# PaddlePaddle/Parakeet

Hardware: AMD Instinct MI355X
Metric: audio samples/sec, FastSpeech2+PWGAN 22.05kHz (higher is better)
Workload: dtype f32 (3-term split-fp16 MFMA, fp32-equivalent; exact-fp32 in roofline.exact_f32); 1 GPU; FastSpeech2+PWG end-to-end (BASELINE config 4 per-GPU share): 32 utterances/GPU x 128 phonemes -> 640 frames -> 163840 samples each, LJSpeech architecture, random-init weights; utterances_per_gpu=32, global_batch=32, minibatch=32, parallelism=dp1 (utterance sharding, no data-path collective)

## Files before the change

parakeet_amd/csrc/ffn_planes.hip:

```cpp
#include "pk_ffn_planes.h"

#include <algorithm>
#include <cmath>
#include <cstdlib>
#include <cstring>

#include "pk_mfma.h"
#include "pk_split.h"

namespace {
constexpr int ROW_B = 16, LO_OFF = 512;

struct Args {
    FfnpConv c;
    int active;
    int nrg;
    int nct;
    long in_blk, out_blk;
};

__device__ __forceinline__ unsigned pow2_neg_h2(int d) {
    const float f = __uint_as_float((unsigned)(127 - min(d, 60)) << 23);
    return __builtin_bit_cast(unsigned, __builtin_amdgcn_cvt_pkrtz(f, f));
}
__device__ __forceinline__ f16x8 h8_of(unsigned u) {
    const u32x4 v = {u, u, u, u};
    return __builtin_bit_cast(f16x8, v);
}

template <int NQ, int KQ, int EPI, int W, int TAPS = FFNP_TAPS, int ABL = 0, bool BF32 = false, int CPT = 6, int ACT = 0>
__global__ __launch_bounds__(64 * W, 2) void k_ffn_planes(Args a) {
    constexpr int THREADS = 64 * W;
    constexpr int HT = TAPS / 2;
    constexpr int SLAB_CH = CPT * THREADS;
    constexpr int KCH = 2 * NQ * 64;
    constexpr int SLAB = SLAB_CH / KCH;
    constexpr int nks = TAPS * KQ;
    constexpr int G = nks / SLAB;
    constexpr int RING = NQ >= 6 ? 6 : 9;
    constexpr bool TIGHT = NQ == 8;
    static_assert(SLAB_CH % KCH == 0 && nks % SLAB == 0 && nks > RING && G >= 3, "shape");
    static_assert(!BF32 || (TAPS == 1 && !TIGHT), "fp32 operand: one tap, the untight loop");
    __shared__ __attribute__((aligned(16))) f16x8 wbuf[3][SLAB_CH];
    __shared__ __attribute__((aligned(16))) float lb[32 * NQ];
    __shared__ float lbs[NQ];
    const int tid = threadIdx.x, lane = tid & 63, wave = tid >> 6;
    const int j = lane & 31, hh = lane >> 5;
    const int xcd = (int)blockIdx.x & 7, k = (int)blockIdx.x >> 3;
    const int rg = (k / a.nct) * 8 + xcd, ct = k % a.nct;
    if (rg >= a.nrg) return;
    for (int i = tid; i < 32 * NQ; i += THREADS) {
        const int h2 = i / (16 * NQ), q = (i / 16) % NQ, r = i % 16;
        lb[i] = a.c.bias ? a.c.bias[ct * (32 * NQ) + 32 * q + mfma_row(r, h2)] : 0.f;
    }
    if (tid < NQ) lbs[tid] = a.c.wscale[ct * NQ + tid];
    const f16x8* wt = reinterpret_cast<const f16x8*>(a.c.w) + (long)ct * ((long)G * SLAB_CH) + tid;
    const int blk = rg * a.active + wave;
    const bool tile_ok = wave < a.active && blk < a.c.nblk;
    f16x8 wreg[CPT];

    if (tile_ok) {
        const int p = blk * FFNP_BLK + j;
        const int rv = a.c.row_utt[p];
        unsigned am[TAPS];
#pragma unroll
        for (int t = 0; t < TAPS; ++t) am[t] = a.c.in_amax[p + t - HT];
        const char* inb = reinterpret_cast<const char*>(a.c.in) + ((long)blk - 1) * a.in_blk;
        unsigned off[TAPS];
#pragma unroll
        for (int t = 0; t < TAPS; ++t) {
            const int q = j + t - HT;
            off[t] = (unsigned)((q + 32) >> 5) * (unsigned)a.in_blk + (unsigned)((q & 31) * ROW_B + hh * 1024);
        }
        f16x8 rhi[RING], rlo[RING];
        auto load_b = [&](int ks) {
            const int kq = ks / TAPS, tap = ks % TAPS, slot = ks % RING;
            if (BF32) {
                const float* src = reinterpret_cast<const float*>(a.c.in) + (long)p * a.c.ldin + 16 * kq + 4 * hh;
                rhi[slot] = ld_h8(reinterpret_cast<const char*>(src));
                rlo[slot] = ld_h8(reinterpret_cast<const char*>(src + 8));
                return;
            }
            const char* src = inb + (off[tap] + (unsigned)(kq * 2048));
            rhi[slot] = ld_h8(src);
            rlo[slot] = ld_h8(src + LO_OFF);
        };
        {
            f16x8 wreg1[CPT];
#pragma unroll
            for (int c = 0; c < CPT; ++c) wreg[c] = wt[c * THREADS];
#pragma unroll
            for (int c = 0; c < CPT; ++c) wreg1[c] = wt[SLAB_CH + c * THREADS];
#pragma unroll
            for (int kk = 0; kk < RING; ++kk) load_b(kk);
            __builtin_amdgcn_sched_barrier(0);
#pragma unroll
            for (int c = 0; c < CPT; ++c) wbuf[0][c * THREADS + tid] = wreg[c];
#pragma unroll
            for (int c = 0; c < CPT; ++c) wbuf[1][c * THREADS + tid] = wreg1[c];
        }
        int ex = amax_exp(am[0]);
#pragma unroll
        for (int t = 1; t < TAPS; ++t) ex = max(ex, amax_exp(am[t]));
        const int kx = PK_BLK_TOP + 127 - ex;
        const float sx = pow2f(kx);
        unsigned fu[TAPS];
#pragma unroll
        for (int t = 0; t < TAPS; ++t) fu[t] = pow2_neg_h2(ex - amax_exp(am[t]));
        f32x16 acc[NQ];
#pragma unroll
        for (int q = 0; q < NQ; ++q)
#pragma unroll
            for (int r = 0; r < 16; ++r) acc[q][r] = 0.f;
        __syncthreads();
#pragma unroll
        for (int g = 0; g < G; ++g) {
            const int NW = g + 2 >= G ? 0 : CPT, HW = TIGHT ? NW / 2 : NW;
#pragma unroll
            for (int c = 0; c < CPT; ++c)
                if (c < HW && !(ABL & (8 | 256))) wreg[c] = wt[(long)(g + 2) * SLAB_CH + c * THREADS];
            __builtin_amdgcn_sched_barrier(0);
            unsigned wo = (g % 3) * SLAB_CH + lane;
            asm volatile("" : "+v"(wo));
            const f16x8* wl = &wbuf[0][0] + wo;
#pragma unroll
            for (int kk = 0; kk < SLAB; ++kk) {
                const int ks = SLAB * g + kk, slot = ks % RING;
                const f16x8 f = h8_of(fu[ks % TAPS]);
                f16x8 bh, bl;
                if (TIGHT) {
                    rhi[slot] *= f;
                    rlo[slot] *= f;
                } else {
                    if (BF32) {
                        const f32x4 v0 = __builtin_bit_cast(f32x4, rhi[slot]), v1 = __builtin_bit_cast(f32x4, rlo[slot]);
                        float v[8];
#pragma unroll
                        for (int e = 0; e < 4; ++e) {
                            v[e] = rv >= 0 ? v0[e] * sx : 0.f;
                            v[4 + e] = rv >= 0 ? v1[e] * sx : 0.f;
                        }
                        split8(v, bh, bl);
                    } else {
                        bh = TAPS == 1 ? rhi[slot] : rhi[slot] * f;
                        bl = TAPS == 1 ? rlo[slot] : rlo[slot] * f;
                    }
                    __builtin_amdgcn_sched_barrier(0);
                    if (!(ABL & 1) && ks + RING < nks) load_b(ks + RING);
                }
                __builtin_amdgcn_sched_barrier(0);
// ... 6 lines not shown
                    acc[q] = mfma16(ah, TIGHT ? rlo[slot] : bl, acc[q]);
                }
                constexpr int AHEAD = NQ == 8 ? 1 : 2;
                __builtin_amdgcn_sched_group_barrier(0x100, 2 * AHEAD, 0);
#pragma unroll
                for (int q = 0; q < NQ; ++q) {
                    if (q + AHEAD < NQ) __builtin_amdgcn_sched_group_barrier(0x100, 2, 0);
                    __builtin_amdgcn_sched_group_barrier(0x008, 3, 0);
                }
                if (TIGHT) {
                    __builtin_amdgcn_sched_barrier(0);
                    if (!(ABL & 1) && ks + RING < nks) load_b(ks + RING);
                    if (kk == 0 && NW > 0 && !(ABL & 8)) {
#pragma unroll
                        for (int c = 0; c < CPT; ++c)
                            if (c < HW) wbuf[(g + 2) % 3][c * THREADS + tid] = wreg[c];
#pragma unroll
                        for (int c = 0; c < CPT; ++c)
                            if (c < NW - HW) wreg[c] = wt[(long)(g + 2) * SLAB_CH + (HW + c) * THREADS];
                    }
                    __builtin_amdgcn_sched_barrier(0);
                }
            }
#pragma unroll
            for (int c = 0; c < CPT; ++c)
                if (c < (TIGHT ? NW - HW : NW) && !(ABL & 8)) {
                    if (ABL & 128) {
                        unsigned keep = __builtin_bit_cast(u32x4, wreg[c])[0];
                        asm volatile("" : "+v"(keep));
                    } else {
                        wbuf[(g + 2) % 3][((TIGHT ? HW : 0) + c) * THREADS + tid] = wreg[c];
                    }
                }
            __syncthreads();
        }
        const float pinv = pow2f(-kx);
        const f32x4* lb4 = reinterpret_cast<const f32x4*>(lb) + hh * (NQ * 4);
        if (EPI == 0) {
            float m3 = __uint_as_float(am[0]);
#pragma unroll
            for (int t = 1; t < TAPS; ++t) m3 = fmaxf(m3, __uint_as_float(am[t]));
            const float hb = fmaf(m3, a.c.c1, a.c.c0);
            const float so = pow2f(blk_scale_exp(__float_as_uint(hb)));
            char* dst = reinterpret_cast<char*>(a.c.out) + (long)blk * a.out_blk + (long)(ct * NQ * 2) * 2048 + j * ROW_B + hh * 1024;
            const bool row_ok = rv >= 0;
#pragma unroll
            for (int q = 0; q < NQ; ++q)
#pragma unroll
                for (int m = 0; m < 2; ++m) {
                    float v[8];
#pragma unroll
                    for (int i = 0; i < 2; ++i) {
                        const f32x4 b4 = lb4[q * 4 + 2 * m + i];
#pragma unroll
                        for (int e = 0; e < 4; ++e) {
                            const float pre = fmaf(acc[q][8 * m + 4 * i + e], pinv * lbs[q], b4[e]);
                            const float t = ACT == 1 ? tanhf(pre) : fmaxf(pre, 0.f);
                            v[4 * i + e] = row_ok ? t : 0.f;
                        }
                    }
                    f16x8 oh, ol;
                    store_pair8(v, so, oh, ol);
                    if ((ABL & 4) && oh[0] != (_Float16)12345.f) continue;
                    st_h8(dst + (2 * q + m) * 2048, oh);
                    st_h8(dst + (2 * q + m) * 2048 + LO_OFF, ol);
                }
            if (ct == 0 && hh == 0) a.c.out_amax[p] = row_ok ? __float_as_uint(hb) : 0u;
// ... 1 lines not shown
            float* yr = a.c.x + (long)p * a.c.ldx + ct * (32 * NQ) + 4 * hh;
#pragma unroll
            for (int q = 0; q < NQ; ++q)
#pragma unroll
                for (int i = 0; i < 4; ++i) {
                    const f32x4 b4 = lb4[q * 4 + i];
                    f32x4 o;
#pragma unroll
                    for (int e = 0; e < 4; ++e) {
                        const float pre = fmaf(acc[q][4 * i + e], pinv * lbs[q], b4[e]);
                        o[e] = ACT == 0 ? pre : (rv >= 0 ? (ACT == 1 ? tanhf(pre) : fmaxf(pre, 0.f)) : 0.f);
                    }
                    *reinterpret_cast<f32x4*>(yr + 32 * q + 8 * i) = o;
                }
        } else {
            float* xr = a.c.x + (long)p * a.c.ldx + ct * (32 * NQ) + 4 * hh;
            f32x4 old[NQ][4];
#pragma unroll
            for (int q = 0; q < NQ; ++q)
#pragma unroll
                for (int i = 0; i < 4; ++i) old[q][i] = (ABL & 4) ? f32x4{0.f, 0.f, 0.f, 0.f} : *reinterpret_cast<const f32x4*>(xr + 32 * q + 8 * i);
#pragma unroll
            for (int q = 0; q < NQ; ++q)
#pragma unroll
                for (int i = 0; i < 4; ++i) {
                    const f32x4 b4 = lb4[q * 4 + i];
                    f32x4 o;
#pragma unroll
                    for (int e = 0; e < 4; ++e) o[e] = old[q][i][e] + fmaf(acc[q][4 * i + e], pinv * lbs[q], b4[e]);
                    if ((ABL & 4) && o[0] != 12345.f) continue;
                    *reinterpret_cast<f32x4*>(xr + 32 * q + 8 * i) = o;
                }
        }
    } else {
#pragma unroll
        for (int c = 0; c < CPT; ++c) wbuf[0][c * THREADS + tid] = wt[c * THREADS];
#pragma unroll
        for (int c = 0; c < CPT; ++c) wbuf[1][c * THREADS + tid] = wt[SLAB_CH + c * THREADS];
        __syncthreads();
#pragma unroll 1
        for (int g = 0; g < G; ++g) {
            if (g + 2 < G) {
#pragma unroll
                for (int c = 0; c < CPT; ++c) wreg[c] = wt[(long)(g + 2) * SLAB_CH + c * THREADS];
#pragma unroll
                for (int c = 0; c < CPT; ++c) wbuf[(g + 2) % 3][c * THREADS + tid] = wreg[c];
            }
            __syncthreads();
        }
    }
}

__global__ __launch_bounds__(256) void k_ffn_ln_planes(const float* __restrict__ x, const float* __restrict__ g,
                                                      const float* __restrict__ b, const int* __restrict__ row_utt, int C,
                                                      float eps, char* __restrict__ out, unsigned* __restrict__ out_amax) {
    const int blk = blockIdx.x, wave = threadIdx.x >> 6, lane = threadIdx.x & 63;
    const int noct = C >> 3;
    const bool on = lane < noct;
    const int kq = lane >> 1, hh = lane & 1;
    const int c0 = 16 * kq + 4 * hh;
    const bool ident = g == nullptr;
    f32x4 ga = {0.f, 0.f, 0.f, 0.f}, gb = ga, ba = ga, bb = ga;
    if (on && !ident) {
        ga = *reinterpret_cast<const f32x4*>(g + c0);
        gb = *reinterpret_cast<const f32x4*>(g + c0 + 8);
        ba = *reinterpret_cast<const f32x4*>(b + c0);
// ... 136 lines not shown
            uint16_t* base = dst + ((size_t)ct * nks + ks) * (2 * nq * 64 * 8);
            for (int q = 0; q < nq; ++q)
                for (int lane = 0; lane < 64; ++lane)
                    for (int e = 0; e < 8; ++e) {
                        const int i = lane & 31, hh = lane >> 5;
                        const int co = ct * 32 * nq + 32 * q + i;
                        const int ci = 16 * kq + 8 * (e >> 2) + 4 * hh + (e & 3);
                        const float w = std::ldexp(kn[((size_t)tap * Cin + ci) * N + co], kw[co / 32]);
                        const uint16_t h = f32_to_f16_rne(w);
                        base[((size_t)(0 * nq + q) * 64 + lane) * 8 + e] = h;
                        base[((size_t)(1 * nq + q) * 64 + lane) * 8 + e] = f32_to_f16_rne(w - f16_to_f32(h));
                    }
        }
    return off;
}

template <bool PROF, class Go>
static int ffnp_ablation(Go& go, bool shape_ok) {
    if constexpr (PROF) {
        static const int abl = pk_prof_env("PK_FFNP_ABLATE") ? atoi(pk_prof_env("PK_FFNP_ABLATE")) : 0;
        if (abl && shape_ok) {
            switch (abl) {
                case 1: return go(k_ffn_planes<4, 96, 1, 4, FFNP_TAPS, 1>);
                case 4: return go(k_ffn_planes<4, 96, 1, 4, FFNP_TAPS, 4>);
                case 8: return go(k_ffn_planes<4, 96, 1, 4, FFNP_TAPS, 8>);
                case 13: return go(k_ffn_planes<4, 96, 1, 4, FFNP_TAPS, 13>);
                case 128: return go(k_ffn_planes<4, 96, 1, 4, FFNP_TAPS, 128>);
                case 256: return go(k_ffn_planes<4, 96, 1, 4, FFNP_TAPS, 256>);
                default: PK_FAIL(PK_EINVAL, "PK_FFNP_ABLATE: 1, 4, 8, 13, 128 or 256 (with PK_FFNP_VARIANT=84)");
            }
        }
    }
    return 1;
}

int ffnp_conv_launch(pk_ctx* ctx, const char* prof_name, const FfnpConv& c) {
    const bool first = c.out != nullptr;
    if (!(first ? (c.Cin == 384 && c.N % (32 * FFNP_NQ1) == 0) : (c.Cin == 1536 && c.N % (32 * FFNP_NQ2) == 0)) || c.nblk <= 0 || !c.w || !c.wscale)
        PK_FAIL(PK_EINVAL, "ffnp_conv_launch: shape (Cin %d, N %d) not built", c.Cin, c.N);
    const int variant = c.variant;
    const bool one = c.w1 && variant == 0 && (long)c.nblk * (c.N / 32) <= c.one_max;
    const bool small = !one && first && c.w4 && (variant / 10 == 4 || (variant / 10 != 8 && c.nblk < FFNP_NQ1_MIN_BLOCKS));
    const int nq = one ? 1 : (first && !small ? FFNP_NQ1 : FFNP_NQ2);
    const int W = one ? 8 : (first ? (small ? 4 : 8) : (variant % 10 == 4 ? 4 : 8));
    Args a;
    a.c = c;
    if (small) a.c.w = c.w4;
    if (one) a.c.w = c.w1;
    a.nct = c.N / (32 * nq);
    a.in_blk = (long)c.Cin * 128;
    a.out_blk = (long)c.N * 128;
    int active = W;
    if (W == 8)
        while (active > 2 && (long)pk_div_up(c.nblk, active) * a.nct < ctx->n_cu) active >>= 1;
    a.active = active;
    a.nrg = pk_div_up(c.nblk, active);
    const int grid = pk_div_up(a.nrg, 8) * 8 * a.nct;
    auto go = [&](auto kern) -> int {
        PK_LAUNCH(ctx, prof_name, kern, dim3(grid), dim3(64 * W), 0, a);
        return PK_OK;
    };
    if (int st = ffnp_ablation<PK_PROFILE_BUILD != 0>(go, !first && W == 4); st != 1) return st;
    if (one) return first ? go(k_ffn_planes<1, 24, 0, 8>) : go(k_ffn_planes<1, 96, 1, 8>);
    if (first) return small ? go(k_ffn_planes<FFNP_NQ2, 24, 0, 4>) : go(k_ffn_planes<FFNP_NQ1, 24, 0, 8>);
    return W == 8 ? go(k_ffn_planes<FFNP_NQ2, 96, 1, 8>) : go(k_ffn_planes<FFNP_NQ2, 96, 1, 4>);
}

int ffnp_linear_launch(pk_ctx* ctx, const char* prof_name, const FfnpConv& c) {
    const int nq = c.ldin ? FFNP_NQ2 : FFNP_NQL;
    if (c.Cin != 384 || c.N % (32 * nq) != 0 || c.nblk <= 0 || !c.w || !c.wscale || !c.x)
        PK_FAIL(PK_EINVAL, "ffnp_linear_launch: shape (Cin %d, N %d) not built", c.Cin, c.N);
    Args a;
    a.c = c;
    a.nct = c.N / (32 * nq);
    a.in_blk = (long)c.Cin * 128;
    a.out_blk = 0;
    int active = 8;
    while (active > 2 && (long)pk_div_up(c.nblk, active) * a.nct < ctx->n_cu) active >>= 1;
    a.active = active;
    a.nrg = pk_div_up(c.nblk, active);
    const int grid = pk_div_up(a.nrg, 8) * 8 * a.nct;
    auto go = [&](auto kern) -> int {
        PK_LAUNCH(ctx, prof_name, kern, dim3(grid), dim3(512), 0, a);
        return PK_OK;
    };
    if (c.ldin) return go(k_ffn_planes<FFNP_NQ2, 24, 1, 8, 1, 0, true>);
    return go(k_ffn_planes<FFNP_NQL, 24, 2, 8, 1>);
}

bool ffnp_conv256_supports(int Cin, int N, int taps) {
    return N == 256 && ((Cin == 384 && (taps == 3 || taps == 5)) || (Cin == 256 && (taps == 3 || taps == 5)));
}
int ffnp_conv256_launch(pk_ctx* ctx, const char* prof_name, const FfnpConv& c, int taps, int act) {
    if (!ffnp_conv256_supports(c.Cin, c.N, taps) || c.nblk <= 0 || !c.w || !c.wscale || (!c.out && !c.x) || act < 1 || act > 2)
        PK_FAIL(PK_EINVAL, "ffnp_conv256_launch: shape (Cin %d, N %d, k %d, act %d) not built", c.Cin, c.N, taps, act);
    if (c.out && act != 1) PK_FAIL(PK_EINVAL, "ffnp_conv256_launch: planes output is built for tanh");
    Args a;
    a.c = c;
    const bool one = c.w1 && c.variant == 0 && (long)c.nblk * (c.N / 32) <= c.one_max;
    if (one) a.c.w = c.w1;
    a.nct = one ? c.N / 32 : c.N / (32 * FFNP_NQ2);
    a.in_blk = (long)c.Cin * 128;
    a.out_blk = (long)c.N * 128;
    int active = 8;
    while (active > 2 && (long)pk_div_up(c.nblk, active) * a.nct < ctx->n_cu) active >>= 1;
    a.active = active;
    a.nrg = pk_div_up(c.nblk, active);
    const int grid = pk_div_up(a.nrg, 8) * 8 * a.nct;
    auto go = [&](auto kern) -> int {
        PK_LAUNCH(ctx, prof_name, kern, dim3(grid), dim3(512), 0, a);
        return PK_OK;
    };
    if (one) {
        if (c.out) {
            if (c.Cin == 256 && taps == 5) return go(k_ffn_planes<1, 16, 0, 8, 5, 0, false, 5, 1>);
            PK_FAIL(PK_EINVAL, "ffnp_conv256_launch: planes output: 256 -> 256, k = 5 only");
        }
        if (act == 1) {
            if (c.Cin == 256 && taps == 5) return go(k_ffn_planes<1, 16, 2, 8, 5, 0, false, 5, 1>);
            PK_FAIL(PK_EINVAL, "ffnp_conv256_launch: tanh rows output: 256 -> 256, k = 5 only");
        }
        if (c.Cin == 384) return taps == 3 ? go(k_ffn_planes<1, 24, 2, 8, 3, 0, false, 6, 2>) : go(k_ffn_planes<1, 24, 2, 8, 5, 0, false, 6, 2>);
        return taps == 3 ? go(k_ffn_planes<1, 16, 2, 8, 3, 0, false, 4, 2>) : go(k_ffn_planes<1, 16, 2, 8, 5, 0, false, 5, 2>);
    }
    if (c.out) {
        if (c.Cin == 256 && taps == 5) return go(k_ffn_planes<4, 16, 0, 8, 5, 0, false, 5, 1>);
        PK_FAIL(PK_EINVAL, "ffnp_conv256_launch: planes output: 256 -> 256, k = 5 only");
    }
    if (act == 1) {
        if (c.Cin == 256 && taps == 5) return go(k_ffn_planes<4, 16, 2, 8, 5, 0, false, 5, 1>);
        PK_FAIL(PK_EINVAL, "ffnp_conv256_launch: tanh rows output: 256 -> 256, k = 5 only");
    }
    if (c.Cin == 384) return taps == 3 ? go(k_ffn_planes<4, 24, 2, 8, 3, 0, false, 6, 2>) : go(k_ffn_planes<4, 24, 2, 8, 5, 0, false, 6, 2>);
    return taps == 3 ? go(k_ffn_planes<4, 16, 2, 8, 3, 0, false, 6, 2>) : go(k_ffn_planes<4, 16, 2, 8, 5, 0, false, 5, 2>);
}

int ffnp_layernorm_launch(pk_ctx* ctx, const float* x, const float* g, const float* b, const int* row_utt, int nblk, int C,
                          float eps, void* out, unsigned* out_amax) {
    if (C % 16 != 0 || C / 8 > 64) PK_FAIL(PK_EINVAL, "ffnp_layernorm_launch: %d channels", C);
    PK_LAUNCH(ctx, g ? "fs2_layernorm_planes" : "fs2_rows_to_planes", k_ffn_ln_planes, dim3(nblk), dim3(256), 0, x, g, b, row_utt, C, eps,
              reinterpret_cast<char*>(out), out_amax);
    return PK_OK;
}
```

parakeet_amd/csrc/fft.hip:

```cpp
#include <algorithm>
#include <cmath>
#include <cstdlib>
#include <cstring>

#include "pk_fft.h"
#include "pk_ffn_planes.h"
#include "pk_gemm.h"
#include "pk_mfma.h"
#include "pk_split.h"

constexpr int FS2_MAX_HEADS = PK_FFT_MAX_HEADS;

namespace {

__global__ void k_build_pe(float* pe, const float* div, int maxlen, int d) {
    const int pos = blockIdx.x;
    for (int c = threadIdx.x; c < d; c += blockDim.x) {
        const float ang = (float)pos * div[c >> 1];
        pe[(long)pos * d + c] = (c & 1) ? cosf(ang) : sinf(ang);
    }
}

__global__ void k_embed(const int* __restrict__ tok, const int* __restrict__ row_utt,
                        const int* __restrict__ row_pos, const float* __restrict__ table,
// ... 1022 lines not shown
    char *hp = nullptr, *fp = nullptr;
    unsigned *hpam = nullptr, *fpam = nullptr;
    if (planes) {
        pk_dbuf* pb[2] = {&h->d_hp, &h->d_fp};
        const int pc[2] = {A, units};
        for (int i = 0; i < 2; ++i) {
            const void* p0 = pb[i]->p;
            PK_TRY(pb[i]->reserve(ffnp_plane_bytes(nblk, pc[i])));
            if (pb[i]->p != p0) PK_HIP(hipMemsetAsync(pb[i]->p, 0, pb[i]->cap, h->ctx->stream));
        }
        PK_TRY(h->d_pam.reserve((size_t)2 * (tl.rows_alloc + 2) * sizeof(unsigned)));
        PK_TRY(zl.add(h->d_pam.p, (size_t)2 * (tl.rows_alloc + 2) * sizeof(unsigned)));
        hp = h->d_hp.as<char>() + (size_t)A * 128;
        fp = h->d_fp.as<char>() + (size_t)units * 128;
        PK_TRY(zl.add(hp + (size_t)nblk * A * 128, (size_t)A * 128));
        PK_TRY(zl.add(fp + (size_t)nblk * units * 128, (size_t)units * 128));
        hpam = h->d_pam.as<unsigned>() + 1;
        fpam = hpam + tl.rows_alloc + 2;
    }
    PK_TRY(zl.launch(h->ctx));
    for (const FftLayer& L : layers) {
        const bool qkv_planes = planes && bounds && !L.concat && L.qkv.wp != (size_t)-1;
        if (qkv_planes) {
            PK_TRY(ffnp_layernorm_launch(h->ctx, x, h->W(L.ln1_g), h->W(L.ln1_b), rv, nblk, A, 1e-5f, hp, hpam));
            FfnpConv c;
            memset(&c, 0, sizeof(c));
            c.nblk = nblk;
            c.row_utt = rv;
            c.w = h->arena16.as<uint16_t>() + L.qkv.wp;
            c.bias = L.qkv.b == (size_t)-1 ? nullptr : h->W(L.qkv.b);
            c.wscale = h->W(L.qkv.wps); c.Cin = A; c.N = 3 * A;
            c.in = hp; c.in_amax = hpam;
            c.x = qkv; c.ldx = 3 * A;
            PK_TRY(ffnp_linear_launch(h->ctx, "fs2_gemm_qkv_planes", c));
        } else {
            PK_TRY(pk_fft_run_layernorm(h, x, L.ln1_g, L.ln1_b, tl, A, hh, ham));
            PK_TRY(pk_fft_run_dense(h, "fs2_gemm_qkv", L.qkv, hh, A, qkv, 3 * A, tl.rows, PK_ACT_NONE, nullptr, 0, nullptr, ham));
        }
        if (bounds) {
            QkvBoundC qc;
            memcpy(qc.c1, L.qkv_c1, sizeof(qc.c1));
            memcpy(qc.c0, L.qkv_c0, sizeof(qc.c0));
            PK_LAUNCH(h->ctx, "fs2_bounds", k_fs2_seg_bounds, dim3(tl.B), dim3(256), 0,
                      qkv_planes ? reinterpret_cast<const float*>(hpam) : ham, tl.d_seg_start(), tl.d_seg_len(), heads, qc, segb,
                      cbnd);
        }
        PK_TRY(pk_fft_run_attention(h, tl, qkv, ctxb, segb));
        if (L.concat) {
            PK_TRY(pk_fft_act_reserve(h->d_cat, tl.rows, A));
            float* t = pk_fft_act_ptr(h->d_cat, A);
            PK_TRY(pk_fft_run_dense(h, "fs2_gemm_attn_out", L.out, ctxb, A, t, A, tl.rows, PK_ACT_NONE, nullptr, 0, nullptr, cbnd));
            PK_TRY(pk_fft_run_dense(h, "fs2_gemm_concat_x", L.cat_x, hh, A, x, A, tl.rows, PK_ACT_NONE, x, A, nullptr, ham));
            PK_TRY(pk_fft_run_dense(h, "fs2_gemm_concat_a", L.cat_a, t, A, x, A, tl.rows, PK_ACT_NONE, x, A, nullptr));
        } else if (qkv_planes && L.out.wp != (size_t)-1) {
            FfnpConv c;
            memset(&c, 0, sizeof(c));
            c.nblk = nblk;
            c.row_utt = rv;
            c.w = h->arena16.as<uint16_t>() + L.out.wp;
            c.wscale = h->W(L.out.wps);
            c.bias = L.out.b == (size_t)-1 ? nullptr : h->W(L.out.b);
            c.Cin = A; c.N = A;
            c.in = ctxb; c.ldin = A; c.in_amax = reinterpret_cast<const unsigned*>(cbnd);
            c.x = x; c.ldx = A;
            PK_TRY(ffnp_linear_launch(h->ctx, "fs2_gemm_attn_out_planes", c));
        } else
        PK_TRY(pk_fft_run_dense(h, "fs2_gemm_attn_out", L.out, ctxb, A, x, A, tl.rows, PK_ACT_NONE, x, A, nullptr, cbnd));
        if (planes) {
            PK_TRY(ffnp_layernorm_launch(h->ctx, x, h->W(L.ln2_g), h->W(L.ln2_b), rv, nblk, A, 1e-5f, hp, hpam));
            FfnpConv c;
            memset(&c, 0, sizeof(c));
            c.nblk = nblk;
            c.row_utt = rv;
            c.w = h->arena16.as<uint16_t>() + L.ffn1.wp;
            c.w4 = L.ffn1.wp4 == (size_t)-1 ? nullptr : h->arena16.as<uint16_t>() + L.ffn1.wp4;
            c.w1 = L.ffn1.wp1 == (size_t)-1 ? nullptr : h->arena16.as<uint16_t>() + L.ffn1.wp1;
            c.bias = L.ffn1.b == (size_t)-1 ? nullptr : h->W(L.ffn1.b);
            c.wscale = h->W(L.ffn1.wps); c.Cin = A; c.N = units;
            c.in = hp; c.in_amax = hpam;
            c.out = fp; c.out_amax = fpam; c.c1 = L.ffn1.c1; c.c0 = L.ffn1.c0;
            c.variant = h->ffnp_variant;
            c.one_max = h->ffn_one_tile_max;
            PK_TRY(ffnp_conv_launch(h->ctx, "fs2_conv_ffn1_planes", c));
            c.w = h->arena16.as<uint16_t>() + L.ffn2.wp;
            c.w4 = nullptr;
            c.w1 = L.ffn2.wp1 == (size_t)-1 ? nullptr : h->arena16.as<uint16_t>() + L.ffn2.wp1;
            c.bias = L.ffn2.b == (size_t)-1 ? nullptr : h->W(L.ffn2.b);
            c.wscale = h->W(L.ffn2.wps); c.Cin = units; c.N = A;
            c.in = fp; c.in_amax = fpam;
            c.out = nullptr; c.out_amax = nullptr;
            c.x = x; c.ldx = A;
            PK_TRY(ffnp_conv_launch(h->ctx, "fs2_conv_ffn2_planes", c));
            continue;
        }
        PK_TRY(pk_fft_run_layernorm(h, x, L.ln2_g, L.ln2_b, tl, A, hh, ham));
        PK_TRY(pk_fft_run_dense(h, "fs2_conv_ffn1", L.ffn1, hh, A, f, units, tl.rows, PK_ACT_RELU, nullptr, 0, rv, ham));
        if (bounds)
            PK_LAUNCH(h->ctx, "fs2_bounds", k_fs2_row_bounds, dim3(pk_div_up(tl.rows, 256)), dim3(256), 0, ham, rv,
                      tl.rows, L.ffn1.pad, L.ffn1.c1, L.ffn1.c0, fbnd);
        PK_TRY(pk_fft_run_dense(h, "fs2_conv_ffn2", L.ffn2, f, units, x, A, tl.rows, PK_ACT_NONE, x, A, nullptr, fbnd));
    }
    PK_TRY(pk_fft_run_layernorm(h, x, after_g, after_b, tl, A, hs_out));
    return PK_OK;
}

constexpr int FFNP_AM_MARGIN = 4;
int pk_fft_planes_buf(pk_fft_core* h, pk_dbuf& buf, pk_dbuf& am, int nblk, int C, char** planes, unsigned** amax) {
    const size_t pb = ffnp_plane_bytes(nblk, C), ab = ((size_t)nblk * FFNP_BLK + 2 * FFNP_AM_MARGIN) * sizeof(unsigned);
    PK_TRY(buf.reserve(pb));
    PK_TRY(am.reserve(ab));
    ZeroItems zl;
    PK_TRY(zl.add(buf.p, (size_t)C * 128));
    PK_TRY(zl.add(buf.as<char>() + (size_t)(nblk + 1) * C * 128, (size_t)C * 128));
    PK_TRY(zl.add(am.p, ab));
    PK_TRY(zl.launch(h->ctx));
    *planes = buf.as<char>() + (size_t)C * 128;
    *amax = am.as<unsigned>() + FFNP_AM_MARGIN;
    return PK_OK;
}

FfnpConv pk_fft_conv256_args(pk_fft_core* h, const Dense& d, int nblk, const int* row_utt, const void* in, const unsigned* in_amax) {
    FfnpConv c;
    memset(&c, 0, sizeof(c));
    c.nblk = nblk;
    c.row_utt = row_utt;
    c.w = h->arena16.as<uint16_t>() + d.wp;
    c.w1 = d.wp1 == (size_t)-1 ? nullptr : h->arena16.as<uint16_t>() + d.wp1;
    c.one_max = h->ffn_one_tile_max;
    c.variant = h->ffnp_variant;
    c.bias = d.b == (size_t)-1 ? nullptr : h->W(d.b);
    c.wscale = h->W(d.wps);
    c.Cin = d.Cin;
    c.N = d.N;
    c.in = in;
    c.in_amax = in_amax;
    return c;
}

int pk_fft_run_postnet(pk_fft_core* h, const char* name, const std::vector<Dense>& postnet, const float* before, int odim,
                       int chans, const Timeline& tl, pk_dbuf& q1, pk_dbuf& q2, float* d_out, const int* out_rowmap,
                       const float* cscale, const float* cshift) {
    const int n = (int)postnet.size();
    PK_TRY(pk_fft_act_reserve(q1, tl.rows, chans));
    PK_TRY(pk_fft_act_reserve(q2, tl.rows, chans));
    const float* in = before;
    int ldin = odim;
    const float* ones = nullptr;
    if (h->math == PK_GEMM_MATH_F16X3 && n > 1) {
        const void* p0 = h->d_ones.p;
        PK_TRY(pk_fft_act_reserve(h->d_ones, tl.rows, 1));
        if (h->d_ones.p != p0)
            PK_HIP(hipMemsetD32Async(reinterpret_cast<hipDeviceptr_t>(h->d_ones.p), 0x3f800000, h->d_ones.cap / 4, h->ctx->stream));
        ones = pk_fft_act_ptr(h->d_ones, 1);
    }
    bool planes = h->math == PK_GEMM_MATH_F16X3 && h->ffn_planes && n >= 4 && tl.rows_alloc % FFNP_BLK == 0 && chans == 256;
    for (int j = 1; j + 1 < n; ++j)
        planes = planes && postnet[j].wp != (size_t)-1 && postnet[j].wps != (size_t)-1 && postnet[j].Cin == 256 && postnet[j].taps == 5;
    for (int j = 0; j < n; ++j) {
        const Dense& d = postnet[j];
        const bool last = j == n - 1;
        float* outb = pk_fft_act_ptr((j & 1) ? q2 : q1, chans);
        if (planes && j == 1) {
// ... 39 lines not shown
            g.C = d_out; g.ldc = odim; g.act = PK_ACT_NONE; g.res = before; g.ldr = odim;
            g.cscale = cscale; g.cshift = cshift; g.out_rowmap = out_rowmap;
        }
        PK_TRY(pk_gemm_launch(h->ctx, name, g));
        in = outb;
        ldin = chans;
    }
    return PK_OK;
}

int pk_fft_embed(pk_fft_core* h, const char* name, const int* d_tok, const Timeline& tl, size_t table, float alpha,
                 float xscale, float* x) {
    PK_LAUNCH(h->ctx, name, k_embed, dim3(tl.rows), dim3(128), 0, d_tok, tl.d_row_utt(), tl.d_row_pos(), h->W(table),
              h->d_pe.as<float>(), alpha, xscale, h->adim, x);
    return PK_OK;
}

int pk_fft_layernorm_rows(pk_fft_core* h, const float* x, size_t g, size_t b, const int* d_row_utt, int rows, int C,
                          float* y, float* amax) {
    if (C % 64 != 0 || C > 64 * LN_MAXPER) PK_FAIL(PK_EUNSUPPORTED, "LayerNorm: %d channels (multiple of 64, <= %d)", C, 64 * LN_MAXPER);
    PK_LAUNCH(h->ctx, "fft_layernorm", k_layernorm, dim3(pk_div_up(rows, 4)), dim3(256), 0, x, h->W(g), h->W(b),
              d_row_utt, rows, C, 1e-5f, y, amax);
    return PK_OK;
}

int pk_fft_set_option(pk_fft_core* h, const char* key, int64_t value, const char* who) {
    if (!h || !key) PK_FAIL(PK_EINVAL, "%s: NULL argument", who);
    if (strcmp(key, "ffn_planes") == 0) h->ffn_planes = value != 0;
    else if (strcmp(key, "ffn_planes_min_blocks") == 0) h->ffn_planes_min_blocks = (int)std::max<int64_t>(0, value);
    else if (strcmp(key, "ffn_one_tile_max") == 0) h->ffn_one_tile_max = (int)std::max<int64_t>(0, std::min<int64_t>(value, 1 << 20));
    else if (strcmp(key, "ffnp_variant") == 0) {
        if (value != 0 && value != 44 && value != 48 && value != 84 && value != 88) PK_FAIL(PK_EINVAL, "%s: ffnp_variant %lld (0, 44, 48, 84, 88)", who, (long long)value);
        h->ffnp_variant = (int)value;
    } else if (strcmp(key, "attn_waves") == 0) {
        if (value != 0 && value != 4 && value != 8) PK_FAIL(PK_EINVAL, "%s: attn_waves %lld (0, 4, 8)", who, (long long)value);
        h->attn_waves = (int)value;
    } else PK_FAIL(PK_EINVAL, "%s: unknown option '%s'", who, key);
    return PK_OK;
}
```

parakeet_amd/csrc/pk_ffn_planes.h:

```cpp
#pragma once
#include <cstdint>
#include <vector>

#include "pk_common.h"

constexpr int FFNP_BLK = 32;
constexpr int FFNP_TAPS = 3;
constexpr int FFNP_NQ1 = 8;
constexpr int FFNP_NQ2 = 4;
constexpr int FFNP_NQL = 6;
constexpr int FFNP_NQ1_MIN_BLOCKS = 256;
constexpr int FFNP_MIN_BLOCKS = 0;

static inline bool ffnp_supports(int A, int units, int taps1, int taps2) {
    return A == 384 && units == 1536 && taps1 == FFNP_TAPS && taps2 == FFNP_TAPS;
}
static inline size_t ffnp_plane_bytes(int nblk, int CH) { return (size_t)(nblk + 2) * CH * 128; }

size_t ffnp_pack(const float* kn, int Cin, int N, int nq, std::vector<uint16_t>& w16, std::vector<float>& wscale,
                 int taps = FFNP_TAPS);
struct FfnpConv {
    const uint16_t* w;
    const uint16_t* w4;
    const uint16_t* w1;
    const float* bias;
    const float* wscale;
    int Cin, N;
    const void* in;
    int ldin;
    const unsigned* in_amax;
    int nblk;
    const int* row_utt;
    void* out;
    unsigned* out_amax;
    float c1, c0;
    float* x;
    int ldx;
    int one_max = 4096;
    int variant = 0;
};
int ffnp_conv_launch(pk_ctx* ctx, const char* prof_name, const FfnpConv& a);
int ffnp_linear_launch(pk_ctx* ctx, const char* prof_name, const FfnpConv& a);

bool ffnp_conv256_supports(int Cin, int N, int taps);
int ffnp_conv256_launch(pk_ctx* ctx, const char* prof_name, const FfnpConv& a, int taps, int act);

int ffnp_layernorm_launch(pk_ctx* ctx, const float* x, const float* g, const float* b, const int* row_utt, int nblk, int C,
                          float eps, void* out, unsigned* out_amax);
```

parakeet_amd/csrc/pk_fft.h:

```cpp
#pragma once
#include <string>
#include <vector>

#include "pk_ffn_planes.h"
#include "pk_gemm.h"

constexpr int PK_FFT_MAX_HEADS = 16;
constexpr int PK_FFT_LN_MAXPER = 8;
constexpr int PK_FFT_LEAD = 8;

struct pk_fft_dense {
    size_t w = 0, b = 0;
    size_t wh = (size_t)-1;
    size_t wp = (size_t)-1;
    size_t wp4 = (size_t)-1;
    size_t wp1 = (size_t)-1;
    size_t wps = (size_t)-1;
    int Cin = 0, N = 0, taps = 1, pad = 0;
    float c1 = 0.f, c0 = 0.f;
};

struct pk_fft_layer {
    size_t ln1_g, ln1_b, ln2_g, ln2_b;
    pk_fft_dense qkv, out, ffn1, ffn2;
// ... 15 lines not shown
};

struct pk_fft_arena {
    std::vector<float>& v;
    std::vector<uint16_t>* v16 = nullptr;
    size_t put(const std::vector<float>& x) {
        size_t o = (v.size() + 3) & ~(size_t)3;
        v.resize(o);
        v.insert(v.end(), x.begin(), x.end());
        return o;
    }
    size_t put16(const std::vector<uint16_t>& x) {
        size_t o = (v16->size() + 7) & ~(size_t)7;
        v16->resize(o);
        v16->insert(v16->end(), x.begin(), x.end());
        return o;
    }
};

struct pk_fft_core {
    pk_ctx* ctx = nullptr;
    int adim = 0, aheads = 0;
    std::vector<float> arena_h;
    pk_dbuf arena;
    std::vector<uint16_t> arena16_h;
    pk_dbuf arena16;
    int math = PK_GEMM_MATH_F16X3;
    bool attn_lds = true;
    bool no_bounds = false;
    bool ffn_planes = true;
    int ffn_planes_min_blocks = 0;
    int ffn_one_tile_max = 4096;
    int ffnp_variant = 0;
    int attn_waves = 0;
    int max_len = 0;
    pk_dbuf d_pe, d_div;
    pk_dbuf d_x, d_h, d_qkv, d_ctx, d_f, d_lnamax, d_cbnd, d_fbnd, d_segb, d_cat;
    pk_dbuf d_hp, d_fp, d_pam;
    pk_dbuf d_ones;
    pk_dbuf d_pnp[2], d_pnam[2];

    const float* W(size_t off) const { return arena.as<float>() + off; }
    void release_core() {
        pk_dbuf* bufs[] = {&arena, &arena16, &d_pe, &d_div, &d_x, &d_h, &d_qkv, &d_ctx, &d_f, &d_lnamax, &d_cbnd,
                           &d_fbnd, &d_segb, &d_cat, &d_hp, &d_fp, &d_pam, &d_ones, &d_pnp[0], &d_pnp[1], &d_pnam[0], &d_pnam[1]};
        for (pk_dbuf* b : bufs) b->release();
    }
};

int pk_fft_act_reserve(pk_dbuf& buf, int rows, int C);
static inline float* pk_fft_act_ptr(const pk_dbuf& buf, int C) { return buf.as<float>() + (size_t)PK_FFT_LEAD * C; }
int pk_fft_build_timeline(pk_ctx* ctx, pk_fft_timeline& tl, const int* lens, int B, int gapr);

int pk_fft_add_dense_kn(pk_fft_arena& ar, const std::vector<float>& kn, const std::vector<float>* bias, int Cin,
                        int taps, int N, pk_fft_dense& d);
int pk_fft_add_linear(pk_fft_arena& ar, const pk_param_map& P, const std::string& base, int Cin, int N,
                      pk_fft_dense& d);
int pk_fft_add_conv(pk_fft_arena& ar, const pk_param_map& P, const std::string& base, int Cout, int Cin, int k,
                    bool bias, pk_fft_dense& d, int planes = 0);
int pk_fft_add_conv_bn(pk_fft_arena& ar, const pk_param_map& P, const std::string& conv_base,
                       const std::string& bn_base, int Cout, int Cin, int k, pk_fft_dense& d, bool conv_bias = false);
int pk_fft_add_vec(pk_fft_arena& ar, const pk_param_map& P, const std::string& name, int n, size_t& off);
int pk_fft_add_stack(pk_fft_arena& ar, const pk_param_map& P, const std::string& prefix, int n_layers, int A,
                     int units, int k, int ff_type, int heads, std::vector<pk_fft_layer>& out, size_t& after_g,
                     size_t& after_b, bool normalize_before = true, bool concat_after = false);
int pk_fft_add_postnet(pk_fft_arena& ar, const pk_param_map& P, const std::string& prefix, int n_layers, int odim,
// ... 28 lines not shown
```

Measured before the change: 125.4 million samples/s.

## Stream FFN plane weights into LDS with a dedicated DMA loader wave

Adds a DMA variant of the FFN-planes GEMM/conv kernel. One extra wave issues global_load_lds transfers of each weight slab straight into the triple-buffered LDS ring and syncs with the compute waves through raw s_barrier, so compute waves no longer stage weights through registers. The B-operand ring is shrunk to free registers, and the launch bound rises to 3 blocks per CU. A per-shape whitelist enables it by default (mode 2) only for selected template instantiations, at the cost of an extra wave per block and hand-managed vmcnt/barrier counts.

```diff
diff --git a/parakeet_amd/csrc/ffn_planes.hip b/parakeet_amd/csrc/ffn_planes.hip
--- a/parakeet_amd/csrc/ffn_planes.hip
+++ b/parakeet_amd/csrc/ffn_planes.hip
@@ -28,8 +28,8 @@
     return __builtin_bit_cast(f16x8, v);
 }
 
-template <int NQ, int KQ, int EPI, int W, int TAPS = FFNP_TAPS, int ABL = 0, bool BF32 = false, int CPT = 6, int ACT = 0>
-__global__ __launch_bounds__(64 * W, 2) void k_ffn_planes(Args a) {
+template <int NQ, int KQ, int EPI, int W, int TAPS = FFNP_TAPS, int ABL = 0, bool BF32 = false, int CPT = 6, int ACT = 0, bool DMA = false>
+__global__ __launch_bounds__(DMA ? 64 * (W + 1) : 64 * W, DMA ? 3 : 2) void k_ffn_planes(Args a) {
     constexpr int THREADS = 64 * W;
     constexpr int HT = TAPS / 2;
     constexpr int SLAB_CH = CPT * THREADS;
@@ -37,10 +37,13 @@
     constexpr int SLAB = SLAB_CH / KCH;
     constexpr int nks = TAPS * KQ;
     constexpr int G = nks / SLAB;
-    constexpr int RING = NQ >= 6 ? 6 : 9;
+    constexpr int RING = DMA && NQ >= 4 ? (NQ >= 6 ? 3 : (EPI == 0 && TAPS == 5 ? 4 : 5)) : (NQ >= 6 ? 6 : 9);
     constexpr bool TIGHT = NQ == 8;
     static_assert(SLAB_CH % KCH == 0 && nks % SLAB == 0 && nks > RING && G >= 3, "shape");
     static_assert(!BF32 || (TAPS == 1 && !TIGHT), "fp32 operand: one tap, the untight loop");
+    constexpr int NDMA = SLAB_CH / 64;
+    constexpr int NBAR = 1 + G;
+    static_assert(!DMA || (ABL == 0 && NDMA <= 63), "loader wave: one slab's DMAs fit the vmcnt counter; no ablations");
     __shared__ __attribute__((aligned(16))) f16x8 wbuf[3][SLAB_CH];
     __shared__ __attribute__((aligned(16))) float lb[32 * NQ];
     __shared__ float lbs[NQ];
@@ -49,6 +52,45 @@
     const int xcd = (int)blockIdx.x & 7, k = (int)blockIdx.x >> 3;
     const int rg = (k / a.nct) * 8 + xcd, ct = k % a.nct;
     if (rg >= a.nrg) return;
+    if (DMA && wave == W) {
+        const f16x8* src = reinterpret_cast<const f16x8*>(a.c.w) + (long)ct * ((long)G * SLAB_CH) + lane;
+        typedef __attribute__((address_space(3))) f16x8 lds_f16x8;
+        lds_f16x8* const l0 = (lds_f16x8*)&wbuf[0][0];
+        auto dma_slab = [&](const f16x8* s, lds_f16x8* d) {
+#pragma unroll
+            for (int i = 0; i < NDMA; ++i)
+                __builtin_amdgcn_global_load_lds((const __attribute__((address_space(1))) void*)(s + i * 64), d + i * 64, 16, 0, 0);
+        };
+        dma_slab(src, l0);
+        asm volatile("s_waitcnt vmcnt(%0)" ::"n"(63 - NDMA) : "memory");
+        dma_slab(src + SLAB_CH, l0 + SLAB_CH);
+        asm volatile("s_waitcnt vmcnt(0)" ::: "memory");
+        __builtin_amdgcn_s_barrier();
+        int b = 2;
+#pragma unroll 1
+        for (int g = 0; g < G; ++g) {
+            if (g + 2 < G) {
+                asm volatile("s_waitcnt vmcnt(%0)" ::"n"(63 - NDMA) : "memory");
+                dma_slab(src + (long)(g + 2) * SLAB_CH, l0 + b * SLAB_CH);
+                b = b == 2 ? 0 : b + 1;
+                asm volatile("s_waitcnt vmcnt(%0)" ::"n"(NDMA) : "memory");
+            } else {
+                asm volatile("s_waitcnt vmcnt(0)" ::: "memory");
+            }
+            __builtin_amdgcn_s_barrier();
+        }
+        static_assert(NBAR == 1 + G, "the loader's barriers: one before the loop, one per iteration");
+        return;
+    }
+    auto slab_barrier = [&]() {
+        if constexpr (DMA) {
+            asm volatile("s_waitcnt lgkmcnt(0)" ::: "memory");
+            __builtin_amdgcn_s_barrier();
+            asm volatile("" ::: "memory");
+        } else {
+            __syncthreads();
+        }
+    };
     for (int i = tid; i < 32 * NQ; i += THREADS) {
         const int h2 = i / (16 * NQ), q = (i / 16) % NQ, r = i % 16;
         lb[i] = a.c.bias ? a.c.bias[ct * (32 * NQ) + 32 * q + mfma_row(r, h2)] : 0.f;
@@ -87,17 +129,21 @@
         };
         {
             f16x8 wreg1[CPT];
-#pragma unroll
-            for (int c = 0; c < CPT; ++c) wreg[c] = wt[c * THREADS];
-#pragma unroll
-            for (int c = 0; c < CPT; ++c) wreg1[c] = wt[SLAB_CH + c * THREADS];
+            if (!DMA) {
+#pragma unroll
+                for (int c = 0; c < CPT; ++c) wreg[c] = wt[c * THREADS];
+#pragma unroll
+                for (int c = 0; c < CPT; ++c) wreg1[c] = wt[SLAB_CH + c * THREADS];
+            }
 #pragma unroll
             for (int kk = 0; kk < RING; ++kk) load_b(kk);
             __builtin_amdgcn_sched_barrier(0);
-#pragma unroll
-            for (int c = 0; c < CPT; ++c) wbuf[0][c * THREADS + tid] = wreg[c];
-#pragma unroll
-            for (int c = 0; c < CPT; ++c) wbuf[1][c * THREADS + tid] = wreg1[c];
+            if (!DMA) {
+#pragma unroll
+                for (int c = 0; c < CPT; ++c) wbuf[0][c * THREADS + tid] = wreg[c];
+#pragma unroll
+                for (int c = 0; c < CPT; ++c) wbuf[1][c * THREADS + tid] = wreg1[c];
+            }
         }
         int ex = amax_exp(am[0]);
 #pragma unroll
@@ -112,10 +158,10 @@
         for (int q = 0; q < NQ; ++q)
 #pragma unroll
             for (int r = 0; r < 16; ++r) acc[q][r] = 0.f;
-        __syncthreads();
+        slab_barrier();
 #pragma unroll
         for (int g = 0; g < G; ++g) {
-            const int NW = g + 2 >= G ? 0 : CPT, HW = TIGHT ? NW / 2 : NW;
+            const int NW = DMA || g + 2 >= G ? 0 : CPT, HW = TIGHT ? NW / 2 : NW;
 #pragma unroll
             for (int c = 0; c < CPT; ++c)
                 if (c < HW && !(ABL & (8 | 256))) wreg[c] = wt[(long)(g + 2) * SLAB_CH + c * THREADS];
@@ -188,7 +234,7 @@
                         wbuf[(g + 2) % 3][((TIGHT ? HW : 0) + c) * THREADS + tid] = wreg[c];
                     }
                 }
-            __syncthreads();
+            slab_barrier();
         }
         const float pinv = pow2f(-kx);
         const f32x4* lb4 = reinterpret_cast<const f32x4*>(lb) + hh * (NQ * 4);
@@ -256,6 +302,10 @@
                     *reinterpret_cast<f32x4*>(xr + 32 * q + 8 * i) = o;
                 }
         }
+    } else if (DMA) {
+        slab_barrier();
+#pragma unroll 1
+        for (int g = 0; g < G; ++g) slab_barrier();
     } else {
 #pragma unroll
         for (int c = 0; c < CPT; ++c) wbuf[0][c * THREADS + tid] = wt[c * THREADS];
@@ -458,6 +508,34 @@
         }
     }
     return 1;
+}
+
+template <int NQ, int KQ, int EPI, int W, int TAPS, bool BF32, int CPT, int ACT>
+constexpr bool ffnp_dma_faster() {
+    return (NQ == 4 && KQ == 96 && EPI == 1 && W == 8) || (NQ == 6 && TAPS == 1) || BF32 || (NQ == 1 && KQ == 96) ||
+           (NQ == 4 && KQ == 24 && EPI == 0 && W == 4) || (NQ == 1 && KQ == 16 && TAPS == 5 && ACT == 2) ||
+           (NQ == 4 && KQ == 16 && EPI == 2 && TAPS == 5 && ACT == 1);
+}
+
+template <int NQ, int KQ, int EPI, int W, int TAPS = FFNP_TAPS, bool BF32 = false, int CPT = 6, int ACT = 0>
+static int ffnp_go(pk_ctx* ctx, const char* prof_name, int grid, const Args& a, int dma) {
+    if constexpr (PK_PROFILE_BUILD != 0 && W == 8 && NQ > 1 && ACT == 0) {
+        static const int abl = pk_prof_env("PK_FFNP_ABLATE") ? atoi(pk_prof_env("PK_FFNP_ABLATE")) : 0;
+        if (abl == 8 || abl == 128 || abl == 256) {
+            if (abl == 8) PK_LAUNCH(ctx, prof_name, (k_ffn_planes<NQ, KQ, EPI, W, TAPS, 8, BF32, CPT, ACT>), dim3(grid), dim3(64 * W), 0, a);
+            if (abl == 128) PK_LAUNCH(ctx, prof_name, (k_ffn_planes<NQ, KQ, EPI, W, TAPS, 128, BF32, CPT, ACT>), dim3(grid), dim3(64 * W), 0, a);
+            if (abl == 256) PK_LAUNCH(ctx, prof_name, (k_ffn_planes<NQ, KQ, EPI, W, TAPS, 256, BF32, CPT, ACT>), dim3(grid), dim3(64 * W), 0, a);
+            return PK_OK;
+        }
+    }
+    if constexpr (ffnp_dma_fits(NQ, W)) {
+        if (dma == 1 || (dma == 2 && ffnp_dma_faster<NQ, KQ, EPI, W, TAPS, BF32, CPT, ACT>())) {
+            PK_LAUNCH(ctx, prof_name, (k_ffn_planes<NQ, KQ, EPI, W, TAPS, 0, BF32, CPT, ACT, true>), dim3(grid), dim3(64 * (W + 1)), 0, a);
+            return PK_OK;
+        }
+    }
+    PK_LAUNCH(ctx, prof_name, (k_ffn_planes<NQ, KQ, EPI, W, TAPS, 0, BF32, CPT, ACT>), dim3(grid), dim3(64 * W), 0, a);
+    return PK_OK;
 }
 
 int ffnp_conv_launch(pk_ctx* ctx, const char* prof_name, const FfnpConv& c) {
@@ -487,9 +565,10 @@
         return PK_OK;
     };
     if (int st = ffnp_ablation<PK_PROFILE_BUILD != 0>(go, !first && W == 4); st != 1) return st;
-    if (one) return first ? go(k_ffn_planes<1, 24, 0, 8>) : go(k_ffn_planes<1, 96, 1, 8>);
-    if (first) return small ? go(k_ffn_planes<FFNP_NQ2, 24, 0, 4>) : go(k_ffn_planes<FFNP_NQ1, 24, 0, 8>);
-    return W == 8 ? go(k_ffn_planes<FFNP_NQ2, 96, 1, 8>) : go(k_ffn_planes<FFNP_NQ2, 96, 1, 4>);
+    const int dma = c.dma;
+    if (one) return first ? ffnp_go<1, 24, 0, 8>(ctx, prof_name, grid, a, dma) : ffnp_go<1, 96, 1, 8>(ctx, prof_name, grid, a, dma);
+    if (first) return small ? ffnp_go<FFNP_NQ2, 24, 0, 4>(ctx, prof_name, grid, a, dma) : ffnp_go<FFNP_NQ1, 24, 0, 8>(ctx, prof_name, grid, a, dma);
+    return W == 8 ? ffnp_go<FFNP_NQ2, 96, 1, 8>(ctx, prof_name, grid, a, dma) : ffnp_go<FFNP_NQ2, 96, 1, 4>(ctx, prof_name, grid, a, dma);
 }
 
 int ffnp_linear_launch(pk_ctx* ctx, const char* prof_name, const FfnpConv& c) {
@@ -506,12 +585,9 @@
     a.active = active;
     a.nrg = pk_div_up(c.nblk, active);
     const int grid = pk_div_up(a.nrg, 8) * 8 * a.nct;
-    auto go = [&](auto kern) -> int {
-        PK_LAUNCH(ctx, prof_name, kern, dim3(grid), dim3(512), 0, a);
-        return PK_OK;
-    };
-    if (c.ldin) return go(k_ffn_planes<FFNP_NQ2, 24, 1, 8, 1, 0, true>);
-    return go(k_ffn_planes<FFNP_NQL, 24, 2, 8, 1>);
+    const int dma = c.dma;
+    if (c.ldin) return ffnp_go<FFNP_NQ2, 24, 1, 8, 1, true>(ctx, prof_name, grid, a, dma);
+    return ffnp_go<FFNP_NQL, 24, 2, 8, 1>(ctx, prof_name, grid, a, dma);
 }
 
 bool ffnp_conv256_supports(int Cin, int N, int taps) {
@@ -533,32 +609,29 @@
     a.active = active;
     a.nrg = pk_div_up(c.nblk, active);
     const int grid = pk_div_up(a.nrg, 8) * 8 * a.nct;
-    auto go = [&](auto kern) -> int {
-        PK_LAUNCH(ctx, prof_name, kern, dim3(grid), dim3(512), 0, a);
-        return PK_OK;
-    };
+    const int dma = c.dma;
     if (one) {
         if (c.out) {
-            if (c.Cin == 256 && taps == 5) return go(k_ffn_planes<1, 16, 0, 8, 5, 0, false, 5, 1>);
+            if (c.Cin == 256 && taps == 5) return ffnp_go<1, 16, 0, 8, 5, false, 5, 1>(ctx, prof_name, grid, a, dma);
             PK_FAIL(PK_EINVAL, "ffnp_conv256_launch: planes output: 256 -> 256, k = 5 only");
         }
         if (act == 1) {
-            if (c.Cin == 256 && taps == 5) return go(k_ffn_planes<1, 16, 2, 8, 5, 0, false, 5, 1>);
+            if (c.Cin == 256 && taps == 5) return ffnp_go<1, 16, 2, 8, 5, false, 5, 1>(ctx, prof_name, grid, a, dma);
             PK_FAIL(PK_EINVAL, "ffnp_conv256_launch: tanh rows output: 256 -> 256, k = 5 only");
         }
-        if (c.Cin == 384) return taps == 3 ? go(k_ffn_planes<1, 24, 2, 8, 3, 0, false, 6, 2>) : go(k_ffn_planes<1, 24, 2, 8, 5, 0, false, 6, 2>);
-        return taps == 3 ? go(k_ffn_planes<1, 16, 2, 8, 3, 0, false, 4, 2>) : go(k_ffn_planes<1, 16, 2, 8, 5, 0, false, 5, 2>);
+        if (c.Cin == 384) return taps == 3 ? ffnp_go<1, 24, 2, 8, 3, false, 6, 2>(ctx, prof_name, grid, a, dma) : ffnp_go<1, 24, 2, 8, 5, false, 6, 2>(ctx, prof_name, grid, a, dma);
+        return taps == 3 ? ffnp_go<1, 16, 2, 8, 3, false, 4, 2>(ctx, prof_name, grid, a, dma) : ffnp_go<1, 16, 2, 8, 5, false, 5, 2>(ctx, prof_name, grid, a, dma);
     }
     if (c.out) {
-        if (c.Cin == 256 && taps == 5) return go(k_ffn_planes<4, 16, 0, 8, 5, 0, false, 5, 1>);
+        if (c.Cin == 256 && taps == 5) return ffnp_go<4, 16, 0, 8, 5, false, 5, 1>(ctx, prof_name, grid, a, dma);
         PK_FAIL(PK_EINVAL, "ffnp_conv256_launch: planes output: 256 -> 256, k = 5 only");
     }
     if (act == 1) {
-        if (c.Cin == 256 && taps == 5) return go(k_ffn_planes<4, 16, 2, 8, 5, 0, false, 5, 1>);
+        if (c.Cin == 256 && taps == 5) return ffnp_go<4, 16, 2, 8, 5, false, 5, 1>(ctx, prof_name, grid, a, dma);
         PK_FAIL(PK_EINVAL, "ffnp_conv256_launch: tanh rows output: 256 -> 256, k = 5 only");
     }
-    if (c.Cin == 384) return taps == 3 ? go(k_ffn_planes<4, 24, 2, 8, 3, 0, false, 6, 2>) : go(k_ffn_planes<4, 24, 2, 8, 5, 0, false, 6, 2>);
-    return taps == 3 ? go(k_ffn_planes<4, 16, 2, 8, 3, 0, false, 6, 2>) : go(k_ffn_planes<4, 16, 2, 8, 5, 0, false, 5, 2>);
+    if (c.Cin == 384) return taps == 3 ? ffnp_go<4, 24, 2, 8, 3, false, 6, 2>(ctx, prof_name, grid, a, dma) : ffnp_go<4, 24, 2, 8, 5, false, 6, 2>(ctx, prof_name, grid, a, dma);
+    return taps == 3 ? ffnp_go<4, 16, 2, 8, 3, false, 6, 2>(ctx, prof_name, grid, a, dma) : ffnp_go<4, 16, 2, 8, 5, false, 5, 2>(ctx, prof_name, grid, a, dma);
 }
 
 int ffnp_layernorm_launch(pk_ctx* ctx, const float* x, const float* g, const float* b, const int* row_utt, int nblk, int C,
diff --git a/parakeet_amd/csrc/fft.hip b/parakeet_amd/csrc/fft.hip
--- a/parakeet_amd/csrc/fft.hip
+++ b/parakeet_amd/csrc/fft.hip
@@ -1078,6 +1078,7 @@
             c.wscale = h->W(L.qkv.wps); c.Cin = A; c.N = 3 * A;
             c.in = hp; c.in_amax = hpam;
             c.x = qkv; c.ldx = 3 * A;
+            c.dma = h->ffn_weight_dma;
             PK_TRY(ffnp_linear_launch(h->ctx, "fs2_gemm_qkv_planes", c));
         } else {
             PK_TRY(pk_fft_run_layernorm(h, x, L.ln1_g, L.ln1_b, tl, A, hh, ham));
@@ -1109,6 +1110,7 @@
             c.Cin = A; c.N = A;
             c.in = ctxb; c.ldin = A; c.in_amax = reinterpret_cast<const unsigned*>(cbnd);
             c.x = x; c.ldx = A;
+            c.dma = h->ffn_weight_dma;
             PK_TRY(ffnp_linear_launch(h->ctx, "fs2_gemm_attn_out_planes", c));
         } else
         PK_TRY(pk_fft_run_dense(h, "fs2_gemm_attn_out", L.out, ctxb, A, x, A, tl.rows, PK_ACT_NONE, x, A, nullptr, cbnd));
@@ -1127,6 +1129,7 @@
             c.out = fp; c.out_amax = fpam; c.c1 = L.ffn1.c1; c.c0 = L.ffn1.c0;
             c.variant = h->ffnp_variant;
             c.one_max = h->ffn_one_tile_max;
+            c.dma = h->ffn_weight_dma;
             PK_TRY(ffnp_conv_launch(h->ctx, "fs2_conv_ffn1_planes", c));
             c.w = h->arena16.as<uint16_t>() + L.ffn2.wp;
             c.w4 = nullptr;
@@ -1174,6 +1177,7 @@
     c.w1 = d.wp1 == (size_t)-1 ? nullptr : h->arena16.as<uint16_t>() + d.wp1;
     c.one_max = h->ffn_one_tile_max;
     c.variant = h->ffnp_variant;
+    c.dma = h->ffn_weight_dma;
     c.bias = d.b == (size_t)-1 ? nullptr : h->W(d.b);
     c.wscale = h->W(d.wps);
     c.Cin = d.Cin;
@@ -1279,6 +1283,9 @@
     else if (strcmp(key, "ffnp_variant") == 0) {
         if (value != 0 && value != 44 && value != 48 && value != 84 && value != 88) PK_FAIL(PK_EINVAL, "%s: ffnp_variant %lld (0, 44, 48, 84, 88)", who, (long long)value);
         h->ffnp_variant = (int)value;
+    } else if (strcmp(key, "ffn_weight_dma") == 0) {
+        if (value < 0 || value > 2) PK_FAIL(PK_EINVAL, "%s: ffn_weight_dma %lld (0, 1, 2)", who, (long long)value);
+        h->ffn_weight_dma = (int)value;
     } else if (strcmp(key, "attn_waves") == 0) {
         if (value != 0 && value != 4 && value != 8) PK_FAIL(PK_EINVAL, "%s: attn_waves %lld (0, 4, 8)", who, (long long)value);
         h->attn_waves = (int)value;
diff --git a/parakeet_amd/csrc/pk_ffn_planes.h b/parakeet_amd/csrc/pk_ffn_planes.h
--- a/parakeet_amd/csrc/pk_ffn_planes.h
+++ b/parakeet_amd/csrc/pk_ffn_planes.h
@@ -38,7 +38,10 @@
     int ldx;
     int one_max = 4096;
     int variant = 0;
+    int dma = 0;
 };
+constexpr int FFNP_DMA_DEFAULT = 2;
+static constexpr bool ffnp_dma_fits(int nq, int waves) { return nq <= 6 && waves >= 4; }
 int ffnp_conv_launch(pk_ctx* ctx, const char* prof_name, const FfnpConv& a);
 int ffnp_linear_launch(pk_ctx* ctx, const char* prof_name, const FfnpConv& a);
 
diff --git a/parakeet_amd/csrc/pk_fft.h b/parakeet_amd/csrc/pk_fft.h
--- a/parakeet_amd/csrc/pk_fft.h
+++ b/parakeet_amd/csrc/pk_fft.h
@@ -71,6 +71,7 @@
     int ffn_planes_min_blocks = 0;
     int ffn_one_tile_max = 4096;
     int ffnp_variant = 0;
+    int ffn_weight_dma = FFNP_DMA_DEFAULT;
     int attn_waves = 0;
     int max_len = 0;
     pk_dbuf d_pe, d_div;
```

New measurement: 125.2 million samples/s, median of 2. Within noise of the previous version (-0.1%).
